# blackle/Megalania

Measured on AMD Instinct MI355X. Metric: SA neighbour-cost evals/s, higher is better.
Workload: dtype u64

## Files before the change

### megalania_amd/csrc/mgl_api.hip

```cpp
#include "mgl_kernels.hip"
#include "mgl_kernels2.hip"
#include "mgl_kernels3.hip"
#include "mgl_kernels4.hip"
#include "mgl_kernels5.hip"
#include "mgl_pbuild.hip"
#include "mgl_index.hip"
#include "mgl_matchfinder.hip"
#include "mgl_optimal.hip"
#include "mgl_adaptive.hip"
#include "mgl_props.hip"
#include "mgl_crossover.hip"
#include "../../include/megalania_hip.h"

#include <math.h>
#include <stdio.h>
#include <stdlib.h>
#include <string.h>
#include <string>
#include <vector>

static const uint16_t k_cost_table[2048] = {
#include "mgl_cost_table.inc"
};

// ... 86 lines not shown
	uint32_t chg_cap = MGL_CHG_CAP;
	uint32_t per_wave_pick, per_wave_rest, pick_waves;
	bool fuse;
	uint32_t fused_lds;
	size_t b2_bytes;
	BigScratch big;
	uint32_t* d_todo2;
	uint4* d_pickstate;
	uint4* d_pickrec;
	bool split_nbr, adaptive;
	bool form_single = false;
	uint32_t* d_counts;
	ApplyBuf ab;
	uint32_t apply_blocks;
	bool incremental_apply;
	bool snapshots;
	Base2 snap_lit, snap_best;
	SnapMeta* d_snap_meta;
	bool parallel_build;
	PBuild pb;
	hipEvent_t ev_begin, ev_end;
	std::vector<hipEvent_t> ev_pool;
	int accept_mode = MGL_ACCEPT_AUTO;
	uint32_t bulk_threshold = 0;
	bool bulk_now = true;
	uint64_t bulk_hold = 0;
	uint64_t blk_done = 0;
	uint64_t blk_imp0 = 0, blk_acc0 = 0;
	BulkBuf bulk;
	BatchBuf batch;
	bool batch_ok = false;
	uint32_t* d_strat_tgt = nullptr;
	uint32_t* d_strat_pre = nullptr;
	bool select_small = false;
	uint32_t* h_bstat = nullptr;
	hipEvent_t ev_bstat = nullptr;
	uint32_t force_xo_nomem = 0;
	uint32_t force_batch_fail = 0;
	uint32_t force_batch_late = 0;
	AcceptLimits lim, lim_max;
	uint64_t batch_early_giveups = 0;
	uint64_t batch_accepts = 0, batch_fallbacks = 0;
	std::vector<uint8_t> mode_log;
	uint32_t force_rollbacks = 0;
	uint64_t bulk_rollbacks = 0;
	bool best_unverified = false;
	uint32_t sim_waves = MGL_SIM_WAVES;
	std::vector<hipEvent_t> ev_sim_pool;
	int64_t time_sim_step = -1;
	bool count_traffic = false;
	unsigned long long* d_traffic = nullptr;
	uint32_t short_looks = 0;
	hipEvent_t ev_val = nullptr;
	int mf_finder = MGL_MF_NEAREST;
	uint32_t mf_depth = MGL_MF_DEF_DEPTH;
	uint32_t mf_built = 0;
	uint32_t* d_mf_off = nullptr;
	uint32_t* d_mf_src = nullptr;
	uint16_t* d_mf_len = nullptr;
	size_t mf_total = 0;
	double mf_ms = 0;
};

static uint64_t ceil_sqrt_u64(uint64_t x)
{
	uint64_t r = (uint64_t)sqrt((double)x);
// ... 194 lines not shown
	if (!sa->snapshots)
		hipLaunchKernelGGL(k_copy_best, dim3(256), dim3(256), 0, sa->stream, (const Control*)sa->base.ctl,
		                   (const mgl_pk*)sa->base.v.slab, sa->d_best, sa->ctx.n);
	hipLaunchKernelGGL(k_apply_chains, dim3(sa->apply_blocks), dim3(MGL_APPLY_THREADS), 0, sa->stream, sa->ctx, accept_b2(sa), sa->base.ctl, accept_ab(sa), sa->lim);
	hipLaunchKernelGGL(k_apply_jobs, dim3(1024), dim3(256), 0, sa->stream, sa->b2, (const Control*)sa->base.ctl, sa->ab, 0, (const uint32_t*)nullptr);
	hipLaunchKernelGGL(k_apply_jobs, dim3(1024), dim3(256), 0, sa->stream, sa->b2, (const Control*)sa->base.ctl, sa->ab, 1, (const uint32_t*)nullptr);
	hipLaunchKernelGGL(k_build_end, dim3(1), dim3(64), sa->build_lds, sa->stream, sa->ctx, sa->b2, sa->base.ctl, sa->snapshots ? 1 : 0, sa->d_counts, sa->adaptive ? 1 : 0, sa->form_single ? 1 : 0);
	HIPCHK(hipGetLastError());
	return MGL_OK;
}
static const bool g_trace = getenv("MGL_TRACE") != nullptr, g_prof_big = getenv("MGL_PROF_BIG") != nullptr;
#define NBR_TRACE(name) do { if (g_trace) { fprintf(stderr, "[mgl] %s\n", name); hipError_t e_ = hipDeviceSynchronize(); if (e_ != hipSuccess) fprintf(stderr, "[mgl] %s -> %s\n", name, hipGetErrorString(e_)); } } while (0)
static hipEvent_t sim_event(mgl_sa* sa, size_t i)
{
	while (sa->ev_sim_pool.size() <= i) {
		hipEvent_t e = nullptr;
		if (hipEventCreate(&e) != hipSuccess) return nullptr;
		sa->ev_sim_pool.push_back(e);
	}
	return sa->ev_sim_pool[i];
}
static uint32_t nbr_slices(const mgl_sa* sa)
{
	const uint32_t K = sa->cfg.neighbours_per_step;
	return (sa->halves >= 2 && K >= 1024) ? sa->halves : 1u;
}
static void launch_targets(mgl_sa* sa, hipStream_t st, uint64_t step_override)
{
	const uint32_t K = sa->cfg.neighbours_per_step;
	const uint64_t* onwalk = sa->incremental ? sa->b2.onwalk : sa->base.v.onwalk;
	const uint32_t nw0 = sa->incremental ? sa->b2.nw0 : (sa->ctx.n + 63u) >> 6;
	hipLaunchKernelGGL(k_rank_blocks, dim3(sa->ctx.strat_nblk), dim3(64), 0, st, onwalk, nw0, sa->d_strat_pre, sa->ctx.strat_nblk);
	hipLaunchKernelGGL(k_rank_scan, dim3(1), dim3(1024), 0, st, sa->d_strat_pre, sa->ctx.strat_nblk);
	hipLaunchKernelGGL(k_targets, dim3((K + 3u) / 4u), dim3(256), 0, st, sa->ctx, onwalk, nw0, (const Control*)sa->base.ctl, sa->cfg.seed, step_override, K, sa->d_strat_tgt);
}
static int launch_targets_ahead(mgl_sa* sa, uint64_t next_gstep)
{
	if (!sa->d_strat_pre || !sa->incremental) return MGL_OK;
	HIPCHK(hipEventRecord(sa->ev_tgt_go, sa->stream));
	HIPCHK(hipStreamWaitEvent(sa->stream2, sa->ev_tgt_go, 0));
	launch_targets(sa, sa->stream2, next_gstep);
	HIPCHK(hipEventRecord(sa->ev_tgt, sa->stream2));
	HIPCHK(hipGetLastError());
	sa->tgt_ahead = 1;
	return MGL_OK;
}
static int launch_neighbours(mgl_sa* sa, uint64_t step_override, bool zero_counts = true)
{
	const uint32_t K = sa->cfg.neighbours_per_step;
	if (sa->d_strat_pre) {
		if (sa->tgt_ahead) HIPCHK(hipStreamWaitEvent(sa->stream, sa->ev_tgt, 0));
		if (sa->tgt_ahead != 1) launch_targets(sa, sa->stream, step_override);
		sa->tgt_ahead = 0;
	}
	if (!sa->incremental) {
		const uint32_t blocks = (K + sa->waves_per_block - 1) / sa->waves_per_block;
		hipLaunchKernelGGL(k_neighbours, dim3(blocks), dim3(64 * sa->waves_per_block), sa->nbr_lds, sa->stream, sa->ctx, sa->base.v,
		                   (const Control*)sa->base.ctl, sa->cfg.seed, step_override, K, sa->nbr, sa->per_wave_bytes,
		                   (const uint32_t*)nullptr, (const uint32_t*)nullptr); NBR_TRACE("k_neighbours");
		HIPCHK(hipGetLastError());
		return MGL_OK;
	}
	if (zero_counts) HIPCHK(hipMemsetAsync(sa->d_counts, 0, 8 * sizeof(uint32_t), sa->stream));
	const uint32_t blocks2 = (K + sa->waves_per_block2 - 1) / sa->waves_per_block2;
	const bool split_now = sa->split_nbr && !sa->form_single;
	const uint32_t sim_lds_regular = ((((sa->ctx.L.total + 31u) >> 5) + 3u) & ~3u) * 4u + sa->chg_cap * 16u;
	if (split_now) {
		const uint32_t slices = nbr_slices(sa);
		HIPCHK(hipEventRecord(sa->ev_fork, sa->stream));
		if (slices >= 2) HIPCHK(hipStreamWaitEvent(sa->stream2, sa->ev_fork, 0));
#if !MGL_TAIL_EARLY
		HIPCHK(hipStreamWaitEvent(sa->stream3, sa->ev_fork, 0));
#endif
		for (uint32_t h = 0; h < slices; h++) {
			const uint32_t j0 = (uint32_t)((uint64_t)K * h / slices), j1 = (uint32_t)((uint64_t)K * (h + 1) / slices);
			hipStream_t st = (h & 1u) ? sa->stream2 : sa->stream;
			if (sa->fuse && !sa->d_prof) {
				hipLaunchKernelGGL((k_neighbours2<false, MGL_NBR_PICKWALK>), dim3(j1 - j0), dim3(64), sa->fused_lds, st, sa->ctx,
				                   sa->b2, sa->base.ctl, sa->cfg.seed, step_override, K, sa->nbr, sa->fused_lds, sa->d_todo, sa->d_counts,
				                   (unsigned long long*)nullptr, sa->big, sa->d_pickrec, j0, j1, sa->d_pickstate); NBR_TRACE("k_neighbours2<false, MGL_NBR_PICKWALK>");
				HIPCHK(hipEventRecord(sa->ev_rest[h], st));
				continue;
			}
			hipLaunchKernelGGL((sa->d_prof ? k_neighbours2<false, MGL_NBR_PICK, true> : k_neighbours2<false, MGL_NBR_PICK>), dim3((j1 - j0 + sa->pick_waves - 1) / sa->pick_waves), dim3(64 * sa->pick_waves),
			                   (MGL_PICK_T_GLOBAL ? 0u : 4096u) + sa->pick_waves * sa->per_wave_pick, st, sa->ctx,
			                   sa->b2, sa->base.ctl, sa->cfg.seed, step_override, K, sa->nbr, sa->per_wave_pick, sa->d_todo, sa->d_counts,
			                   sa->d_prof, sa->big, sa->d_pickrec, j0, j1, sa->d_pickstate); NBR_TRACE("k_neighbours2<false, MGL_NBR_PICK>");
			hipLaunchKernelGGL((k_neighbours2<false, MGL_NBR_REST>), dim3(j1 - j0), dim3(64), sa->per_wave_rest, st, sa->ctx,
			                   sa->b2, sa->base.ctl, sa->cfg.seed, step_override, K, sa->nbr, sa->per_wave_rest, sa->d_todo, sa->d_counts,
			                   g_prof_big ? (unsigned long long*)nullptr : sa->d_prof, sa->big, sa->d_pickrec, j0, j1, sa->d_pickstate); NBR_TRACE("k_neighbours2<false, MGL_NBR_REST>");
			HIPCHK(hipEventRecord(sa->ev_rest[h], st));
		}
		HIPCHK(hipGetLastError());
		for (uint32_t h = 0; h < slices; h++) {
			const uint32_t j0 = (uint32_t)((uint64_t)K * h / slices), j1 = (uint32_t)((uint64_t)K * (h + 1) / slices);
			HIPCHK(hipStreamWaitEvent(sa->stream3, sa->ev_rest[h], 0));
			if (sa->time_sim_step >= 0 && h < 2) HIPCHK(hipEventRecord(sim_event(sa, 4 * (size_t)sa->time_sim_step + 2 * h), sa->stream3));
			if (sa->count_traffic)
				hipLaunchKernelGGL(k_sim<true>, dim3(j1 - j0), dim3(64 * sa->sim_waves), sim_lds_regular, sa->stream3, sa->ctx, sa->b2, sa->base.ctl,
				                   sa->nbr, sa->big, j0, j1, sa->d_traffic);
			else
				hipLaunchKernelGGL(k_sim<false>, dim3(j1 - j0), dim3(64 * sa->sim_waves), sim_lds_regular, sa->stream3, sa->ctx, sa->b2, sa->base.ctl,
				                   sa->nbr, sa->big, j0, j1, (unsigned long long*)nullptr);
			NBR_TRACE("k_sim");
			if (sa->time_sim_step >= 0 && h < 2) HIPCHK(hipEventRecord(sim_event(sa, 4 * (size_t)sa->time_sim_step + 2 * h + 1), sa->stream3));
		}
		HIPCHK(hipEventRecord(sa->ev_sim, sa->stream3));
		for (uint32_t h = 1; h < slices; h += 2) HIPCHK(hipStreamWaitEvent(sa->stream, sa->ev_rest[h], 0));
	}
	if (!sa->split_nbr || sa->form_single) {
		hipLaunchKernelGGL((k_neighbours2<false, MGL_NBR_FULL>), dim3(blocks2), dim3(64 * sa->waves_per_block2), sa->nbr2_lds, sa->stream, sa->ctx,
		                   sa->b2, sa->base.ctl, sa->cfg.seed, step_override, K, sa->nbr, sa->per_wave2, sa->d_todo, sa->d_counts,
		                   sa->d_prof, sa->big, sa->d_pickrec, 0u, K, sa->d_pickstate); NBR_TRACE("k_neighbours2<false, MGL_NBR_FULL>");
	}
	const uint32_t bigblocks = sa->big.slots < 1024u ? sa->big.slots : 1024u;
	const uint32_t big_lds = 4096u + sa->per_wave2 + 12u * MGL_BIG_CAP + MGL_COOP_BYTES;
	hipLaunchKernelGGL((k_neighbours2<true, MGL_NBR_FULL>), dim3(bigblocks), dim3(64 * sa->big_waves), big_lds, sa->stream, sa->ctx,
	                   sa->b2, sa->base.ctl, sa->cfg.seed, step_override, K, sa->nbr, sa->per_wave2, sa->d_todo2, sa->d_counts + 1,
	                   g_prof_big ? sa->d_prof : (unsigned long long*)nullptr, sa->big, split_now ? sa->d_pickrec : (uint4*)nullptr, 0u, K, sa->d_pickstate); NBR_TRACE("k_neighbours2<true, MGL_NBR_FULL>");
#if !MGL_TAIL_EARLY
	if (split_now) HIPCHK(hipStreamWaitEvent(sa->stream, sa->ev_sim, 0));
#endif
	const uint32_t blocks = (K + sa->waves_per_block - 1) / sa->waves_per_block;
	hipLaunchKernelGGL(k_neighbours, dim3(blocks < 256u ? blocks : 256u), dim3(64 * sa->waves_per_block), sa->nbr_lds, sa->stream, sa->ctx, sa->base.v,
	                   (const Control*)sa->base.ctl, sa->cfg.seed, step_override, K, sa->nbr, sa->per_wave_bytes,
	                   (const uint32_t*)sa->d_todo2, (const uint32_t*)(sa->d_counts + 1)); NBR_TRACE("k_neighbours");
#if MGL_TAIL_EARLY
	if (split_now) HIPCHK(hipStreamWaitEvent(sa->stream, sa->ev_sim, 0));
// ... 12 lines not shown
static int export_slab(mgl_sa* sa, const mgl_pk* d_slab, mgl_packet* packets)
{
	hipLaunchKernelGGL(k_export, dim3(1024), dim3(256), 0, sa->stream, d_slab, sa->d_aos, sa->n);
	HIPCHK(hipGetLastError());
	HIPCHK(hipMemcpyAsync(packets, sa->d_aos, sizeof(mgl_packet) * (size_t)sa->n, hipMemcpyDeviceToHost, sa->stream));
	HIPCHK(hipStreamSynchronize(sa->stream));
	return MGL_OK;
}

extern "C" void mgl_sa_destroy(mgl_sa* sa)
{
	if (!sa) return;
	(void)hipSetDevice(sa->device);
	if (sa->stream) (void)hipStreamSynchronize(sa->stream);
	dfree(sa->d_data); dfree(sa->d_bucket_off); dfree(sa->d_bucket_pos); dfree(sa->d_bucket_nx); dfree(sa->d_quad_pos); dfree(sa->d_quad_nx); dfree(sa->d_cost_tbl);
	dfree(sa->d_quad_rank); dfree(sa->d_quad_run); dfree(sa->d_oct_pos);
	for (int i = 0; i < 6; i++) { if (i != 0 && i != 2) { dfree(sa->d_xpos[i]); dfree(sa->d_xrank[i]); dfree(sa->d_xrun[i]); } dfree(sa->d_xnxb[i]); } dfree(sa->d_oct_rank); dfree(sa->d_oct_run);
	dfree(sa->d_hex_pos); dfree(sa->d_hex_rank); dfree(sa->d_hex_run); dfree(sa->d_oct_nx8); dfree(sa->d_hex_nx8);
	free_base(sa->base); free_base(sa->scratch);
	if (!sa->snapshots) dfree(sa->d_best);
	dfree(sa->nbr.cost); dfree(sa->nbr.ndiffs); dfree(sa->nbr.walked); dfree(sa->nbr.win); dfree(sa->nbr.win2); dfree(sa->nbr.dpos);
	dfree(sa->bulk.ckey); dfree(sa->bulk.cwin); dfree(sa->bulk.taken); dfree(sa->bulk.cstate); dfree(sa->bulk.cflags); dfree(sa->bulk.hdr);
	dfree(sa->nbr.dold); dfree(sa->nbr.dnew);
	dfree(sa->d_aos); dfree(sa->d_cum); dfree(sa->d_final_probs);
	free_b2(sa->b2, false);
	free_b2(sa->snap_lit, true); free_b2(sa->snap_best, true); dfree(sa->d_snap_meta);
	dfree(sa->pb.exits); dfree(sa->pb.entry); dfree(sa->pb.gexits); dfree(sa->pb.gentry); dfree(sa->pb.gsum); dfree(sa->pb.ch_map); dfree(sa->pb.ch_vs); dfree(sa->pb.ch_pk); dfree(sa->pb.ch_state); dfree(sa->pb.tf_ctx); dfree(sa->pb.tf_dist); dfree(sa->pb.tf_pk);
	dfree(sa->pb.st_in); dfree(sa->pb.hist); dfree(sa->pb.stage); dfree(sa->pb.stage_n); dfree(sa->pb.stage_over); dfree(sa->pb.acc); dfree(sa->pb.seg_off); dfree(sa->pb.unres);
	dfree(sa->d_todo); dfree(sa->d_prof);
	dfree(sa->big.sim_hdr); dfree(sa->big.sim_keys); dfree(sa->big.sim_pos);
	dfree(sa->big.ins_key); dfree(sa->big.rem_key); dfree(sa->big.ins_pos); dfree(sa->big.rem_pos); dfree(sa->big.uctx);
	if (sa->h_bstat) (void)hipHostFree(sa->h_bstat);
	if (sa->ev_bstat) (void)hipEventDestroy(sa->ev_bstat);
	dfree(sa->big.cont); dfree(sa->d_traffic); dfree(sa->d_strat_pre); dfree(sa->d_strat_tgt);
	{
		BatchBuf& bt = sa->batch;
		dfree(bt.hdr); dfree(bt.cl); dfree(bt.jpos); dfree(bt.jnew); dfree(bt.jold); dfree(bt.st_ikey); dfree(bt.st_rkey); dfree(bt.st_ipos);
		dfree(bt.st_rpos); dfree(bt.ops); dfree(bt.ins_cl); dfree(bt.rem_cl); dfree(bt.acc); dfree(bt.runs);
		dfree(bt.cnt_i); dfree(bt.cnt_r); dfree(bt.off_i); dfree(bt.off_r); dfree(bt.cur_i); dfree(bt.cur_r); dfree(bt.touched);
		dfree(bt.bk_ipos); dfree(bt.bk_rpos); dfree(bt.bk_ibit); dfree(bt.bk_icl); dfree(bt.bk_rcl);
	}
	for (hipEvent_t e : sa->ev_sim_pool) if (e) (void)hipEventDestroy(e);
	dfree(sa->d_todo2); dfree(sa->d_counts); dfree(sa->d_pickrec); dfree(sa->d_pickstate);
	dfree(sa->lim.why); dfree(sa->ab.hdr); dfree(sa->ab.ins_key); dfree(sa->ab.rem_key); dfree(sa->ab.ins_pos); dfree(sa->ab.rem_pos);
	dfree(sa->ab.tctx); dfree(sa->ab.scratch_pos); dfree(sa->ab.scratch_ev);
	dfree(sa->ab.span_pos); dfree(sa->ab.span_ev); dfree(sa->ab.jobs_b); dfree(sa->ab.jobs_c);
	dfree(sa->d_mf_off); dfree(sa->d_mf_src); dfree(sa->d_mf_len);
	dfree(sa->d_topk_pk); dfree(sa->d_topk_cost); dfree(sa->d_small); dfree(sa->d_sub_offs); dfree(sa->d_sub_lens);
	for (hipEvent_t e : sa->ev_pool) (void)hipEventDestroy(e);
	if (sa->ev_begin) (void)hipEventDestroy(sa->ev_begin);
	if (sa->ev_end) (void)hipEventDestroy(sa->ev_end);
	if (sa->stream2) (void)hipStreamDestroy(sa->stream2);
	if (sa->stream3) (void)hipStreamDestroy(sa->stream3);
	for (auto& e : sa->ev_rest) if (e) (void)hipEventDestroy(e);
	if (sa->ev_sim) (void)hipEventDestroy(sa->ev_sim);
	if (sa->ev_val) (void)hipEventDestroy(sa->ev_val);
	if (sa->ev_fork) (void)hipEventDestroy(sa->ev_fork);
	if (sa->ev_tgt) (void)hipEventDestroy(sa->ev_tgt);
	if (sa->ev_tgt_go) (void)hipEventDestroy(sa->ev_tgt_go);
	if (sa->ev_join) (void)hipEventDestroy(sa->ev_join);
	if (sa->stream) (void)hipStreamDestroy(sa->stream);
	delete sa;
}

static int create_impl(mgl_sa* sa, const uint8_t* data, size_t n)
{
	HIPCHK(hipSetDevice(sa->device));
// ... 354 lines not shown
			}
		}
		if (getenv("MGL_SIMW")) { const int w = atoi(getenv("MGL_SIMW")); if (w == 1 || w == 2 || w == 4 || w == 8) sa->sim_waves = (uint32_t)w; }
		sa->adaptive = sa->split_nbr && getenv("MGL_NO_ADAPT") == nullptr;
		sa->form_single = !sa->split_nbr;
		sa->pick_waves = getenv("MGL_PICK_WAVES") ? (uint32_t)atoi(getenv("MGL_PICK_WAVES")) : 0u;
		if (sa->pick_waves != 1 && sa->pick_waves != 2 && sa->pick_waves != 4 && sa->pick_waves != 8) sa->pick_waves = 0;
		{
			uint32_t best_w = 1, best_resident = 0;
			for (uint32_t w = 1; w <= 8; w *= 2) {
				const uint32_t bytes = (MGL_PICK_T_GLOBAL ? 0u : 4096u) + w * sa->per_wave_pick;
				if (bytes > 160u * 1024u) break;
				const uint32_t resident = (160u * 1024u / ((bytes + 1279u) / 1280u * 1280u)) * w;
				if (resident > best_resident) { best_resident = resident; best_w = w; }
			}
			if (n > (1u << 20)) best_w = 1;
			if (sa->pick_waves == 0 || (MGL_PICK_T_GLOBAL ? 0u : 4096u) + sa->pick_waves * sa->per_wave_pick > 160u * 1024u) sa->pick_waves = best_w;
		}
		HIPCHK(hipFuncSetAttribute((const void*)k_sim<false>, hipFuncAttributeMaxDynamicSharedMemorySize, 96 * 1024));
		HIPCHK(hipFuncSetAttribute((const void*)k_sim<true>, hipFuncAttributeMaxDynamicSharedMemorySize, 96 * 1024));
		HIPCHK(hipMalloc(&sa->d_traffic, sizeof(unsigned long long) * 2));
		HIPCHK(hipMemset(sa->d_traffic, 0, sizeof(unsigned long long) * 2));
		HIPCHK(hipFuncSetAttribute((const void*)k_build, hipFuncAttributeMaxDynamicSharedMemorySize, (int)sa->build_lds));
		HIPCHK(hipFuncSetAttribute((const void*)k_build_end, hipFuncAttributeMaxDynamicSharedMemorySize, (int)sa->build_lds));
	}

	if (!(sa->cfg.flags & MGL_F_POSITION_TARGETS)) {
		sa->ctx.strat_nblk = (uint32_t)((n + 4095u) / 4096u);
		HIPCHK(hipMalloc(&sa->d_strat_pre, sizeof(uint32_t) * (sa->ctx.strat_nblk + 2u)));
		HIPCHK(hipMemset(sa->d_strat_pre, 0, sizeof(uint32_t) * (sa->ctx.strat_nblk + 2u)));
		sa->ctx.strat_pre = sa->d_strat_pre;
		HIPCHK(hipMalloc(&sa->d_strat_tgt, sizeof(uint32_t) * sa->cfg.neighbours_per_step));
		sa->ctx.strat_tgt = sa->d_strat_tgt;
	}
	sa->sqrt_thresh = ceil_sqrt_u64(sa->cfg.iters_per_epoch);
	sa->bulk_threshold = getenv("MGL_BULK_THRESHOLD") ? (uint32_t)atoi(getenv("MGL_BULK_THRESHOLD"))
	                     : sa->batch_ok ? 2u : (n <= (1u << 20) ? 16u : n <= (1u << 24) ? 32u : 128u);
	if (sa->bulk_threshold == 0) sa->bulk_threshold = 1;

	hipLaunchKernelGGL(k_fill_literal, dim3(1024), dim3(256), 0, sa->stream, sa->base.v.slab, sa->ctx.n);
	if (!sa->d_best) HIPCHK(hipMalloc(&sa->d_best, sizeof(mgl_pk) * n));
	hipLaunchKernelGGL(k_fill_literal, dim3(1024), dim3(256), 0, sa->stream, sa->d_best, sa->ctx.n);
	HIPCHK(hipGetLastError());
	int rc = rebuild_base(sa, 0);
	if (rc) return rc;
	if (sa->incremental && sa->snapshots && (rc = launch_snapshot(sa, sa->snap_lit, 0, 0, 0))) return rc;
	HIPCHK(hipStreamSynchronize(sa->stream));
	{
		Control c0;
		HIPCHK(hipMemcpy(&c0, sa->base.ctl, sizeof c0, hipMemcpyDeviceToHost));
		if (c0.error_flags) return fail(MGL_EDEVICE, "mgl_sa_create: building the base structures of the all-literal slab failed");
	}
	return MGL_OK;
}

extern "C" mgl_sa* mgl_sa_create(const uint8_t* data, size_t n, mgl_properties props, const mgl_sa_config* cfg)
{
	if (!data || n == 0 || !cfg) { fail(MGL_EINVAL, "mgl_sa_create: bad data/size/config"); return nullptr; }
	if (n > MGL_MAX_INPUT) { fail(MGL_EINVAL, "mgl_sa_create: input larger than 176 000 000 bytes is not supported"); return nullptr; }
	if (props.lc + props.lp > 4 || props.pb > 4 || props.lc > 8) { fail(MGL_EINVAL, "mgl_sa_create: unsupported lc/lp/pb"); return nullptr; }
	mgl_sa* sa = new (std::nothrow) mgl_sa();
	if (!sa) { fail(MGL_ENOMEM, "mgl_sa_create: out of host memory"); return nullptr; }
	sa->cfg = *cfg;
	sa->props = props;
	sa->n = (uint32_t)n;
	sa->device = cfg->device;
// ... 1337 lines not shown
	case 10: {
		uint32_t v[16];
		*bytes = sizeof v;
		if (cap_bytes < sizeof v) return fail(MGL_ERANGE, "mgl_debug_dump: buffer too small");
		HIPCHK(hipMemcpy(v, sa->d_counts + 8, sizeof(uint32_t) * 8, hipMemcpyDeviceToHost));
		HIPCHK(hipMemcpy(v + 8, sa->d_counts, sizeof(uint32_t) * 8, hipMemcpyDeviceToHost));
		memcpy(out, v, sizeof v);
		return MGL_OK;
	}
	case 14: src = sa->ab.hdr; sz = sa->ab.hdr ? sizeof(uint32_t) * 16 : 0; break;
	case 16: src = sa->base.ctl; sz = sizeof(Control); break;
	case 15: src = sa->d_pickrec; sz = sa->d_pickrec ? sizeof(uint4) * sa->cfg.neighbours_per_step : 0; break;
	case 18: src = sa->d_quad_pos; sz = sizeof(uint32_t) * (sa->n - 1); break;
	case 19: src = sa->d_quad_nx; sz = sizeof(uint16_t) * (sa->n - 1); break;
	case 12: src = sa->d_bucket_off; sz = sizeof(uint32_t) * 65537; break;
	case 13: src = sa->d_bucket_pos; sz = sizeof(uint32_t) * (sa->n - 1); break;
	case 30: case 31: case 32: case 33: case 34: case 35: src = sa->d_xpos[what - 30]; sz = sizeof(uint32_t) * (sa->n - 1); break;
	case 40: case 41: case 42: case 43: case 44: case 45: src = sa->d_xrank[what - 40]; sz = src ? sizeof(uint32_t) * (sa->n - 1) : 0; break;
	case 50: case 51: case 52: case 53: case 54: case 55: src = sa->d_xrun[what - 50]; sz = src ? sizeof(uint32_t) * (sa->n - 1) : 0; break;
	case 60: case 61: case 62: case 63: case 64: case 65: src = sa->d_xnxb[what - 60]; sz = sa->n - 1; break;
	case 70: src = sa->d_oct_pos; sz = sizeof(uint32_t) * (sa->n - 1); break;
	case 71: src = sa->d_oct_rank; sz = sizeof(uint32_t) * (sa->n - 1); break;
	case 72: src = sa->d_oct_run; sz = sizeof(uint32_t) * (sa->n - 1); break;
	case 73: src = sa->d_oct_nx8; sz = sizeof(uint64_t) * (sa->n - 1); break;
	case 74: src = sa->d_hex_pos; sz = sizeof(uint32_t) * (sa->n - 1); break;
	case 75: src = sa->d_hex_rank; sz = sizeof(uint32_t) * (sa->n - 1); break;
	case 76: src = sa->d_hex_run; sz = sizeof(uint32_t) * (sa->n - 1); break;
	case 77: src = sa->d_hex_nx8; sz = sizeof(uint64_t) * (sa->n - 1); break;
	case 23: src = sa->nbr.cost; sz = sizeof(uint64_t) * sa->cfg.neighbours_per_step; break;
	case 24: src = sa->nbr.ndiffs; sz = sizeof(uint32_t) * sa->cfg.neighbours_per_step; break;
	case 25: src = sa->nbr.walked; sz = sizeof(uint32_t) * sa->cfg.neighbours_per_step; break;
	case 22: src = sa->nbr.win2; sz = sizeof(uint32_t) * sa->cfg.neighbours_per_step; break;
	case 21: src = sa->nbr.win; sz = sizeof(uint32_t) * 2 * sa->cfg.neighbours_per_step; break;
	case 11: src = sa->pb.acc; sz = sa->pb.acc ? sizeof(unsigned long long) * 8 : 0; break;
	default: return fail(MGL_EINVAL, "mgl_debug_dump: unknown selector");
	}
	*bytes = sz;
	if (sz > cap_bytes) return fail(MGL_ERANGE, "mgl_debug_dump: buffer too small");
	HIPCHK(hipMemcpy(out, src, sz, hipMemcpyDeviceToHost));
	if (what == 84) HIPCHK(hipMemset(sa->lim.why, 0, sizeof(uint32_t)));
	return MGL_OK;
}

extern "C" int mgl_debug_set(mgl_sa* sa, uint32_t key, uint64_t value)
{
	if (sa && key == 5) {
		sa->force_batch_late = (uint32_t)(value >> 32);
		sa->force_batch_fail = (uint32_t)value;
		if (sa->force_batch_late && !sa->force_batch_fail) sa->force_batch_fail = 1;
		return MGL_OK;
	}
	if (sa && key == 6) {
		const uint32_t id = (uint32_t)(value & 0xFFu);
		const uint64_t v = value >> 8;
		if (!sa->incremental || !sa->lim.why) return fail(MGL_EINVAL, "mgl_debug_set: no in-place accept on this handle");
		HIPCHK(hipSetDevice(sa->device));
		HIPCHK(hipStreamSynchronize(sa->stream));
		if (id == 0) {
			if (v) return fail(MGL_EINVAL, "mgl_debug_set: limit id 0 takes value 0 (restore the defaults)");
			for (uint32_t i = 1; i < MGL_LIM_COUNT; i++) sa->lim.v[i] = i == MGL_LIM_SOFT_REACH ? 0u : sa->lim_max.v[i];
		} else {
			if (id >= MGL_LIM_COUNT || v > sa->lim_max.v[id]) return fail(MGL_EINVAL, "mgl_debug_set: unknown limit, or a value above the compiled / allocated one");
			sa->lim.v[id] = (uint32_t)v;
		}
		HIPCHK(hipMemset(sa->lim.why, 0, sizeof(uint32_t)));
		return MGL_OK;
	}
	if (sa && key == 4) {
		if (!sa->d_traffic) return fail(MGL_EINVAL, "mgl_debug_set: no split neighbour evaluation on this handle");
		sa->count_traffic = value != 0;
		return MGL_OK;
	}
	if (!sa) return fail(MGL_EINVAL, "null handle");
	if (key == 0) { sa->ctx.diag_stop = (uint32_t)value; return MGL_OK; }
	if (key == 1) { sa->pb.force_fix = (uint32_t)value; return MGL_OK; }
	if (key == 2) {
		if (value < 8 || value > sa->chg_cap || (value & 7u)) return fail(MGL_EINVAL, "mgl_debug_set: list capacity must be a multiple of 8 within the allocated one");
		sa->big.chg_cap = (uint32_t)value;
		return MGL_OK;
	}
	if (key == 7) {
		if (value != 1 && value != 2 && value != MGL_BIG_WAVES) return fail(MGL_EINVAL, "mgl_debug_set: 1, 2 or MGL_BIG_WAVES wavefronts");
		sa->big_waves = (uint32_t)value;
		return MGL_OK;
	}
	if (key == 8) { sa->force_xo_nomem = (uint32_t)value; return MGL_OK; }
	if (key == 3) { sa->force_rollbacks = (uint32_t)value; return MGL_OK; }
	return fail(MGL_EINVAL, "mgl_debug_set: unknown key");
}

#include "mgl_exchange.inc"
```

### megalania_amd/csrc/mgl_kernels2.hip

```cpp
#include "mgl_base2.h"


struct BitAcc {
	uint32_t word;
	uint64_t bits;
};
__device__ __forceinline__ void bitacc_move(BitAcc& a, uint64_t* arr, uint32_t new_word, uint32_t lane)
{
	if (new_word == a.word) return;
	if (lane == 0) arr[a.word] = a.bits;
	for (uint32_t z = a.word + 1 + lane; z < new_word; z += 64) arr[z] = 0;
	a.word = new_word; a.bits = 0;
}

__device__ void build_body(const DevCtx& c, const Base2& b, Control* ctl, int check_cost)
{
	extern __shared__ __attribute__((aligned(16))) unsigned char smem[];
	uint16_t* T = (uint16_t*)smem;
	uint16_t* probs = (uint16_t*)(smem + 4096);
	uint32_t* cnt = (uint32_t*)(smem + 4096 + (size_t)b.ck_elems * 2);
	uint32_t* off = cnt + b.ck_elems;
	const uint32_t lane = threadIdx.x;
	const uint32_t total = c.L.total;
	if (check_cost && !ctl->accepted_flag) return;
// ... 826 lines not shown
	if (c.diag_stop == 1) { if (lane == 0) { out.cost[j] = MGL_INVALID_COST; out.ndiffs[j] = 0; out.walked[j] = first; } return; }
	if (MODE == MGL_NBR_REST && FUSED) {
		mutated = (hand->flags & MGL_HAND_MUTATED) != 0; second_set = (hand->flags & MGL_HAND_SECOND) != 0;
		if (mutated) {
			m_first = hand->m_first; m_second = hand->m_second;
			journal_set(jn, pos, first, m_first, lane);
			if (second_set) journal_set(jn, pos + 1, hand->second, m_second, lane);
		}
	} else if (!(BIG && resumed) && pos + 1 < c.n && (nbr_draw(rng) % 2u) == 0) {
		const mgl_pk second = uni64(b.slab[pos + 1]);
		const uint32_t ft = mgl_pk_type(first), flen = mgl_pk_len(first);
		const uint32_t st = mgl_pk_type(second), slen = mgl_pk_len(second), sdist = mgl_pk_dist(second);
		if ((ft == MGL_LONG_REP || ft == MGL_MATCH) && flen > 2) {
			m_second = mgl_pack(ft, mgl_pk_dist(first), flen - 1);
			m_first = MGL_PK_LITERAL;
			if (MODE == MGL_NBR_PICK && FUSED) hand->second = uni64(second);
			if (MODE != MGL_NBR_PICK) { journal_set(jn, pos, first, m_first, lane); journal_set(jn, pos + 1, second, m_second, lane); }
			second_set = true; mutated = true;
		} else if ((ft == MGL_LITERAL || ft == MGL_SHORT_REP) && (st == MGL_MATCH || st == MGL_LONG_REP)) {
			uint32_t rep_start = pos - (st == MGL_LONG_REP ? mgl_dist_at(&nb, sdist) : sdist);
			if (slen < MGL_MAX_MATCH && rep_start > 0 && rep_start <= pos && win_byte(win, pos) == c.data[rep_start - 1]) {
				m_first = mgl_pack(st, sdist, slen + 1);
				if (MODE != MGL_NBR_PICK) journal_set(jn, pos, first, m_first, lane);
				mutated = true;
			}
		}
	}
	enum { P_MODEL, P_SIM, P_TOPK, P_WALK, P_OUT };
	uint32_t phase = mutated ? P_WALK : P_MODEL;
	if (MODE == MGL_NBR_PICK && FUSED) {
		hand->m_first = uni64(m_first); hand->m_second = uni64(m_second); hand->rng_n = uni(rng.n);
		hand->flags = (mutated ? MGL_HAND_MUTATED : 0u) | (second_set ? MGL_HAND_SECOND : 0u);
	}
	if (MODE == MGL_NBR_PICK && mutated) return;
	TopkPlan plan;
	if (MODE == MGL_NBR_PICK) {
		if (PROF) pick_prof_mark(&pp, 0, lane);
		if (MGL_PICK_BATCH) topk_plan_make(plan, c, nb, lane);
		if (PROF) pick_prof_mark(&pp, 1, lane);
	}
	if (MODE == MGL_NBR_REST && c.diag_stop != 0 && c.diag_stop != 4 && c.diag_stop < 40) return;
	bool pick_is_mutation = !mutated;
	uint32_t pick_pos = pos;
	mgl_pk pick_inc = first;
	bool pick_best = false;
	bool have_pick = false;
	mgl_pk picked_pk = 0, resume_old = 0;
	uint32_t sim_limit = MGL_POS_INF;
	bool sim_overlay = false;
	int64_t delta = 0;
	bool generate_failed = false, sim_deferred = false, walk_long = false;
	uint32_t npicks = 0;
	uint32_t count = 0;
	uint32_t walked = 0;
	uint32_t wend = 0;
	uint32_t wsoft = 0xFFFFFFFFu, taint = 0xFu, dep = 0u;
	bool first_packet = true;
	uint32_t guard = 0;
	if (BIG && resumed) {
		bs.pos = uni(crec[9]); bs.ctx_state = uni(crec[10]);
		bs.dists[0] = uni(crec[11]); bs.dists[1] = uni(crec[12]); bs.dists[2] = uni(crec[13]); bs.dists[3] = uni(crec[14]);
		count = uni(crec[15]); walked = uni(crec[16]); npicks = uni(crec[17]); wsoft = uni(crec[18]); taint = uni(crec[19]); dep = uni(crec[20]);
		rng.n = uni(crec[21]); guard = uni(crec[22]); jn.count = uni(crec[23]); ch.n_ins = uni(crec[24]); ch.n_rem = uni(crec[25]);
		const uint32_t fl = uni(crec[26]);
		pick_best = (fl & 1u) != 0; second_set = (fl & 2u) != 0;
		pick_inc = (mgl_pk)uni(crec[28]) | ((mgl_pk)uni(crec[29]) << 32);
		resume_old = (mgl_pk)uni(crec[30]) | ((mgl_pk)uni(crec[31]) << 32);
// ... 304 lines not shown
		if (lane == 0) {
			out.dpos[(size_t)j * MGL_MAX_DIFFS + nd] = jn.pos[i];
			out.dold[(size_t)j * MGL_MAX_DIFFS + nd] = jn.old[i];
			out.dnew[(size_t)j * MGL_MAX_DIFFS + nd] = jn.neu[i];
		}
		nd++;
	}
	if (lane == 0) { if (!sim_deferred) out.cost[j] = total; out.ndiffs[j] = nd; out.walked[j] = walked; out.win[2u * j] = pos; out.win[2u * j + 1u] = wend; out.win2[j] = (wsoft < wend ? wsoft : wend) | (dep << 31); }
	if (prof_acc && lane == 0)
		prof_acc[32 + j] = ((__builtin_readcyclecounter() - t_begin) & 0xFFFFFFFFFFull) |
		                   ((unsigned long long)((ch.n_ins + ch.n_rem) & 0xFFFu) << 40) | ((unsigned long long)(walked & 0xFFFu) << 52);
}

template <bool BIG, int MODE, bool PROF = false>
__global__ void __launch_bounds__((MODE == MGL_NBR_PICK ? 512 : (BIG ? 64 * MGL_BIG_WAVES : 64)), (MODE == MGL_NBR_FULL ? (BIG ? 1 : MGL_NBR_WAVES_PER_SIMD) : (MODE == MGL_NBR_REST ? MGL_REST_WAVES_PER_SIMD : 4)))  k_neighbours2(DevCtx c, Base2 b, Control* ctl, uint64_t seed,
                                                     uint64_t step_override, uint32_t K, NbrOut out, uint32_t per_wave_bytes,
                                                     uint32_t* todo, uint32_t* todo_count, unsigned long long* prof_acc,
                                                     BigScratch big, uint4* pickrec, uint32_t j_base, uint32_t j_end, uint4* pickstate)
{
	const uint32_t waves = blockDim.x >> 6;
	if (BIG && blockIdx.x >= *big.todo_in_count) return;
	extern __shared__ __attribute__((aligned(16))) unsigned char smem[];
	uint16_t* T = (uint16_t*)smem;
	if (BIG && threadIdx.x == 0) { CoopCmd* cmd = coop_cmd(smem, per_wave_bytes); cmd->gen = 0; cmd->op = MGL_COOP_SIM; }
	if ((MODE == MGL_NBR_PICK || MODE == MGL_NBR_PICKWALK) && MGL_PICK_T_GLOBAL) {
		T = const_cast<uint16_t*>(c.cost_tbl);
	} else if (MODE != MGL_NBR_REST) {
		for (uint32_t i = threadIdx.x; i < 256; i += blockDim.x) reinterpret_cast<uint4*>(T)[i] = reinterpret_cast<const uint4*>(c.cost_tbl)[i];
		__syncthreads();
	}
	const uint32_t lane = threadIdx.x & 63u, wid = threadIdx.x >> 6;
	if constexpr (MODE == MGL_NBR_PICKWALK) {
		static_assert(!BIG && !PROF, "the fused instance is a regular launch without stage marks");
		PickHand hand;
		hand.target = 0; hand.rng_n = 0; hand.ctx_state = 0; hand.dists[0] = hand.dists[1] = hand.dists[2] = hand.dists[3] = 0;
		hand.first = hand.second = hand.m_first = hand.m_second = 0; hand.flags = 0;
		nbr2_one<false, MGL_NBR_PICK, false, true>(c, b, ctl, seed, step_override, K, out, per_wave_bytes, todo, todo_count, nullptr, big, pickrec, j_base, j_end, pickstate, smem, T,
		                                           blockIdx.x, lane, 0u, &hand);
		wave_sync();
		nbr2_one<false, MGL_NBR_REST, false, true>(c, b, ctl, seed, step_override, K, out, per_wave_bytes, todo, todo_count, nullptr, big, pickrec, j_base, j_end, pickstate, smem, T,
		                                           blockIdx.x, lane, 0u, &hand);
	} else if (BIG) {
		if (wid != 0) { coop_helpers(c, b, big, prof_acc, smem, per_wave_bytes, T, lane, wid); return; }
		const uint32_t n = *big.todo_in_count;
		for (uint32_t unit = blockIdx.x; unit < n; unit += gridDim.x)
			nbr2_one<BIG, MODE, PROF>(c, b, ctl, seed, step_override, K, out, per_wave_bytes, todo, todo_count, prof_acc, big, pickrec, j_base, j_end, pickstate, smem, T, unit, lane, 0u);
		if (lane == 0) { CoopCmd* cmd = coop_cmd(smem, per_wave_bytes); cmd->op = MGL_COOP_EXIT; cmd->gen = cmd->gen + 1u; }
		__syncthreads();
	} else {
		nbr2_one<BIG, MODE, PROF>(c, b, ctl, seed, step_override, K, out, per_wave_bytes, todo, todo_count, prof_acc, big, pickrec, j_base, j_end, pickstate, smem, T,
		                    blockIdx.x * waves + wid, lane, wid);
	}
}


#ifndef MGL_SIM_WAVES
#define MGL_SIM_WAVES 2u
#endif
#define MGL_SIM_WAVES_MAX 8u
struct SimShared {
	uint16_t* T;
	uint32_t* dyn;
	unsigned long long* sum;
	uint32_t* nu_many;
};
template <bool COUNT>
__device__ __forceinline__ void sim_one(const DevCtx& c, const Base2& b, Control* ctl, const NbrOut& out, const BigScratch& big, const uint4* hdrs,
                                        uint32_t j, const SimShared& sh, unsigned long long* traffic_ctr)
{
	const uint4 hdr = hdrs[j];
	if (hdr.x == 0xFFFFFFFFu) return;
	const uint32_t cap = big.chg_cap;
	uint32_t* s_bits = sh.dyn;
	uint32_t* s_pos = sh.dyn + ((((c.L.total + 31u) >> 5) + 3u) & ~3u);
// ... 61 lines not shown


__global__ void __launch_bounds__(64) k_rank_blocks(const uint64_t* onwalk, uint32_t nw0, uint32_t* pre, uint32_t nblk)
{
	const uint32_t blk = blockIdx.x, lane = threadIdx.x;
	if (blk >= nblk) return;
	const uint32_t w = blk * 64u + lane;
	unsigned long long v = w < nw0 ? (unsigned long long)__popcll(onwalk[w]) : 0ull;
	v = wave_sum64(v);
	if (lane == 0) pre[blk + 1u] = (uint32_t)v;
}
__global__ void __launch_bounds__(1024) k_rank_scan(uint32_t* pre, uint32_t nblk)
{
	__shared__ uint32_t s_w[16], s_base;
	const uint32_t tid = threadIdx.x, lane = tid & 63u, wid = tid >> 6;
	if (tid == 0) { s_base = 0; pre[0] = 0; }
	__syncthreads();
	for (uint32_t base = 0; base < nblk; base += blockDim.x) {
		const uint32_t i = base + tid;
		const uint32_t v = i < nblk ? pre[i + 1u] : 0u;
		uint32_t incl = v;
		for (int o = 1; o < 64; o <<= 1) { const uint32_t t = (uint32_t)__shfl_up((int)incl, o, 64); if ((int)lane >= o) incl += t; }
		if (lane == 63) s_w[wid] = incl;
		__syncthreads();
		uint32_t bsum = s_base;
		for (uint32_t q = 0; q < wid; q++) bsum += s_w[q];
		if (i < nblk) pre[i + 1u] = bsum + incl;
		__syncthreads();
		if (tid == blockDim.x - 1u) s_base = bsum + incl;
		__syncthreads();
	}
}

__global__ void __launch_bounds__(256) k_targets(DevCtx c, const uint64_t* onwalk, uint32_t nw0, const Control* ctl, uint64_t seed, uint64_t step_override,
                                                 uint32_t K, uint32_t* tgt)
{
	const uint32_t j = blockIdx.x * (blockDim.x >> 6) + (threadIdx.x >> 6), lane = threadIdx.x & 63u;
	if (j >= K) return;
	const uint64_t gstep = step_override != ~0ull ? step_override : ctl->gstep;
	const uint32_t t = stratified_target(onwalk, nw0, c.strat_pre, c.strat_nblk, c.strat_pre[c.strat_nblk], K, j, mgl_rng_draw(mgl_rng_key(seed, gstep, j), 0), lane);
	if (lane == 0) tgt[j] = t;
}
```

Baseline: 15.87 million.

## Predict picking neighbours and launch them first in fused neighbour kernel

Adds a cheap prediction in k_targets of whether each neighbour will take the expensive pick path, then a k_pick_order kernel that partitions each slice so predicted-picking neighbours come first in block order. The fused PICKWALK kernel reads this permutation to map block index to neighbour unit, aiming to schedule long-running blocks early and reduce tail imbalance. It costs an extra slab read per target, an extra kernel launch, and per-step scans, and it changes the pickstate argument semantics in the fused path.

```diff
diff --git a/megalania_amd/csrc/mgl_api.hip b/megalania_amd/csrc/mgl_api.hip
--- a/megalania_amd/csrc/mgl_api.hip
+++ b/megalania_amd/csrc/mgl_api.hip
@@ -142,6 +142,8 @@
 	bool batch_ok = false;
 	uint32_t* d_strat_tgt = nullptr;
 	uint32_t* d_strat_pre = nullptr;
+	unsigned char* d_pick_hint = nullptr;
+	uint32_t* d_pick_order = nullptr;
 	bool select_small = false;
 	uint32_t* h_bstat = nullptr;
 	hipEvent_t ev_bstat = nullptr;
@@ -402,7 +404,12 @@
 	const uint32_t nw0 = sa->incremental ? sa->b2.nw0 : (sa->ctx.n + 63u) >> 6;
 	hipLaunchKernelGGL(k_rank_blocks, dim3(sa->ctx.strat_nblk), dim3(64), 0, st, onwalk, nw0, sa->d_strat_pre, sa->ctx.strat_nblk);
 	hipLaunchKernelGGL(k_rank_scan, dim3(1), dim3(1024), 0, st, sa->d_strat_pre, sa->ctx.strat_nblk);
-	hipLaunchKernelGGL(k_targets, dim3((K + 3u) / 4u), dim3(256), 0, st, sa->ctx, onwalk, nw0, (const Control*)sa->base.ctl, sa->cfg.seed, step_override, K, sa->d_strat_tgt);
+	hipLaunchKernelGGL(k_targets, dim3((K + 3u) / 4u), dim3(256), 0, st, sa->ctx, sa->b2, onwalk, nw0, (const Control*)sa->base.ctl, sa->cfg.seed, step_override, K, sa->d_strat_tgt,
+	                   sa->d_pick_hint);
+	if (sa->d_pick_order) {
+		const uint32_t slices = nbr_slices(sa);
+		hipLaunchKernelGGL(k_pick_order, dim3(slices), dim3(1024), 0, st, (const unsigned char*)sa->d_pick_hint, sa->d_pick_order, K, slices);
+	}
 }
 static int launch_targets_ahead(mgl_sa* sa, uint64_t next_gstep)
 {
@@ -443,12 +450,12 @@
 		HIPCHK(hipStreamWaitEvent(sa->stream3, sa->ev_fork, 0));
 #endif
 		for (uint32_t h = 0; h < slices; h++) {
-			const uint32_t j0 = (uint32_t)((uint64_t)K * h / slices), j1 = (uint32_t)((uint64_t)K * (h + 1) / slices);
+			const uint32_t j0 = mgl_slice_bound(K, h, slices), j1 = mgl_slice_bound(K, h + 1, slices);
 			hipStream_t st = (h & 1u) ? sa->stream2 : sa->stream;
 			if (sa->fuse && !sa->d_prof) {
 				hipLaunchKernelGGL((k_neighbours2<false, MGL_NBR_PICKWALK>), dim3(j1 - j0), dim3(64), sa->fused_lds, st, sa->ctx,
 				                   sa->b2, sa->base.ctl, sa->cfg.seed, step_override, K, sa->nbr, sa->fused_lds, sa->d_todo, sa->d_counts,
-				                   (unsigned long long*)nullptr, sa->big, sa->d_pickrec, j0, j1, sa->d_pickstate); NBR_TRACE("k_neighbours2<false, MGL_NBR_PICKWALK>");
+				                   (unsigned long long*)nullptr, sa->big, sa->d_pickrec, j0, j1, (uint4*)sa->d_pick_order); NBR_TRACE("k_neighbours2<false, MGL_NBR_PICKWALK>");
 				HIPCHK(hipEventRecord(sa->ev_rest[h], st));
 				continue;
 			}
@@ -463,7 +470,7 @@
 		}
 		HIPCHK(hipGetLastError());
 		for (uint32_t h = 0; h < slices; h++) {
-			const uint32_t j0 = (uint32_t)((uint64_t)K * h / slices), j1 = (uint32_t)((uint64_t)K * (h + 1) / slices);
+			const uint32_t j0 = mgl_slice_bound(K, h, slices), j1 = mgl_slice_bound(K, h + 1, slices);
 			HIPCHK(hipStreamWaitEvent(sa->stream3, sa->ev_rest[h], 0));
 			if (sa->time_sim_step >= 0 && h < 2) HIPCHK(hipEventRecord(sim_event(sa, 4 * (size_t)sa->time_sim_step + 2 * h), sa->stream3));
 			if (sa->count_traffic)
@@ -542,7 +549,7 @@
 	dfree(sa->big.ins_key); dfree(sa->big.rem_key); dfree(sa->big.ins_pos); dfree(sa->big.rem_pos); dfree(sa->big.uctx);
 	if (sa->h_bstat) (void)hipHostFree(sa->h_bstat);
 	if (sa->ev_bstat) (void)hipEventDestroy(sa->ev_bstat);
-	dfree(sa->big.cont); dfree(sa->d_traffic); dfree(sa->d_strat_pre); dfree(sa->d_strat_tgt);
+	dfree(sa->big.cont); dfree(sa->d_traffic); dfree(sa->d_strat_pre); dfree(sa->d_strat_tgt); dfree(sa->d_pick_hint); dfree(sa->d_pick_order);
 	{
 		BatchBuf& bt = sa->batch;
 		dfree(bt.hdr); dfree(bt.cl); dfree(bt.jpos); dfree(bt.jnew); dfree(bt.jold); dfree(bt.st_ikey); dfree(bt.st_rkey); dfree(bt.st_ipos);
@@ -963,6 +970,11 @@
 		sa->ctx.strat_pre = sa->d_strat_pre;
 		HIPCHK(hipMalloc(&sa->d_strat_tgt, sizeof(uint32_t) * sa->cfg.neighbours_per_step));
 		sa->ctx.strat_tgt = sa->d_strat_tgt;
+		if (sa->incremental && sa->split_nbr && getenv("MGL_NO_ORDER") == nullptr) {
+			HIPCHK(hipMalloc(&sa->d_pick_hint, sa->cfg.neighbours_per_step));
+			HIPCHK(hipMemset(sa->d_pick_hint, 1, sa->cfg.neighbours_per_step));
+			HIPCHK(hipMalloc(&sa->d_pick_order, sizeof(uint32_t) * sa->cfg.neighbours_per_step));
+		}
 	}
 	sa->sqrt_thresh = ceil_sqrt_u64(sa->cfg.iters_per_epoch);
 	sa->bulk_threshold = getenv("MGL_BULK_THRESHOLD") ? (uint32_t)atoi(getenv("MGL_BULK_THRESHOLD"))
@@ -2366,12 +2378,15 @@
 	case 25: src = sa->nbr.walked; sz = sizeof(uint32_t) * sa->cfg.neighbours_per_step; break;
 	case 22: src = sa->nbr.win2; sz = sizeof(uint32_t) * sa->cfg.neighbours_per_step; break;
 	case 21: src = sa->nbr.win; sz = sizeof(uint32_t) * 2 * sa->cfg.neighbours_per_step; break;
+	case 26: src = sa->d_pick_hint; sz = src ? sa->cfg.neighbours_per_step : 0; break;
+	case 27: src = sa->d_pick_order; sz = src ? sizeof(uint32_t) * sa->cfg.neighbours_per_step : 0; break;
+	case 28: src = sa->d_pickstate; sz = src ? sizeof(uint4) * 2 * sa->cfg.neighbours_per_step : 0; break;
 	case 11: src = sa->pb.acc; sz = sa->pb.acc ? sizeof(unsigned long long) * 8 : 0; break;
 	default: return fail(MGL_EINVAL, "mgl_debug_dump: unknown selector");
 	}
 	*bytes = sz;
 	if (sz > cap_bytes) return fail(MGL_ERANGE, "mgl_debug_dump: buffer too small");
-	HIPCHK(hipMemcpy(out, src, sz, hipMemcpyDeviceToHost));
+	if (sz) HIPCHK(hipMemcpy(out, src, sz, hipMemcpyDeviceToHost));
 	if (what == 84) HIPCHK(hipMemset(sa->lim.why, 0, sizeof(uint32_t)));
 	return MGL_OK;
 }
@@ -2419,6 +2434,24 @@
 		return MGL_OK;
 	}
 	if (key == 8) { sa->force_xo_nomem = (uint32_t)value; return MGL_OK; }
+	if (key == 9) {
+		if (!sa->d_pick_order) return fail(MGL_EINVAL, "mgl_debug_set: no launch order on this handle");
+		const uint32_t K = sa->cfg.neighbours_per_step, slices = nbr_slices(sa);
+		std::vector<unsigned char> h(K);
+		uint64_t x = value;
+		for (uint32_t j = 0; j < K; j++) {
+			x = x * 6364136223846793005ull + 1442695040888963407ull;
+			h[j] = value == 0 ? 0 : value == 1 ? 1 : value == 2 ? (unsigned char)(j & 1u) : (unsigned char)((x >> 40) % 3u);
+		}
+		HIPCHK(hipSetDevice(sa->device));
+		HIPCHK(hipStreamSynchronize(sa->stream));
+		HIPCHK(hipStreamSynchronize(sa->stream2));
+		HIPCHK(hipMemcpy(sa->d_pick_hint, h.data(), K, hipMemcpyHostToDevice));
+		hipLaunchKernelGGL(k_pick_order, dim3(slices), dim3(1024), 0, sa->stream, (const unsigned char*)sa->d_pick_hint, sa->d_pick_order, K, slices);
+		HIPCHK(hipGetLastError());
+		HIPCHK(hipStreamSynchronize(sa->stream));
+		return MGL_OK;
+	}
 	if (key == 3) { sa->force_rollbacks = (uint32_t)value; return MGL_OK; }
 	return fail(MGL_EINVAL, "mgl_debug_set: unknown key");
 }
diff --git a/megalania_amd/csrc/mgl_kernels2.hip b/megalania_amd/csrc/mgl_kernels2.hip
--- a/megalania_amd/csrc/mgl_kernels2.hip
+++ b/megalania_amd/csrc/mgl_kernels2.hip
@@ -882,7 +882,10 @@
 		hand->m_first = uni64(m_first); hand->m_second = uni64(m_second); hand->rng_n = uni(rng.n);
 		hand->flags = (mutated ? MGL_HAND_MUTATED : 0u) | (second_set ? MGL_HAND_SECOND : 0u);
 	}
-	if (MODE == MGL_NBR_PICK && mutated) return;
+	if (MODE == MGL_NBR_PICK && mutated) {
+		if (!FUSED && lane == 0) reinterpret_cast<uint32_t*>(pickstate)[8u * j + 7u] = 1u;
+		return;
+	}
 	TopkPlan plan;
 	if (MODE == MGL_NBR_PICK) {
 		if (PROF) pick_prof_mark(&pp, 0, lane);
@@ -1253,14 +1256,16 @@
 	const uint32_t lane = threadIdx.x & 63u, wid = threadIdx.x >> 6;
 	if constexpr (MODE == MGL_NBR_PICKWALK) {
 		static_assert(!BIG && !PROF, "the fused instance is a regular launch without stage marks");
+		const uint32_t* const order = reinterpret_cast<const uint32_t*>(pickstate);
+		const uint32_t unit = order != nullptr ? order[j_base + blockIdx.x] - j_base : blockIdx.x;
 		PickHand hand;
 		hand.target = 0; hand.rng_n = 0; hand.ctx_state = 0; hand.dists[0] = hand.dists[1] = hand.dists[2] = hand.dists[3] = 0;
 		hand.first = hand.second = hand.m_first = hand.m_second = 0; hand.flags = 0;
-		nbr2_one<false, MGL_NBR_PICK, false, true>(c, b, ctl, seed, step_override, K, out, per_wave_bytes, todo, todo_count, nullptr, big, pickrec, j_base, j_end, pickstate, smem, T,
-		                                           blockIdx.x, lane, 0u, &hand);
+		nbr2_one<false, MGL_NBR_PICK, false, true>(c, b, ctl, seed, step_override, K, out, per_wave_bytes, todo, todo_count, nullptr, big, pickrec, j_base, j_end, nullptr, smem, T,
+		                                           unit, lane, 0u, &hand);
 		wave_sync();
-		nbr2_one<false, MGL_NBR_REST, false, true>(c, b, ctl, seed, step_override, K, out, per_wave_bytes, todo, todo_count, nullptr, big, pickrec, j_base, j_end, pickstate, smem, T,
-		                                           blockIdx.x, lane, 0u, &hand);
+		nbr2_one<false, MGL_NBR_REST, false, true>(c, b, ctl, seed, step_override, K, out, per_wave_bytes, todo, todo_count, nullptr, big, pickrec, j_base, j_end, nullptr, smem, T,
+		                                           unit, lane, 0u, &hand);
 	} else if (BIG) {
 		if (wid != 0) { coop_helpers(c, b, big, prof_acc, smem, per_wave_bytes, T, lane, wid); return; }
 		const uint32_t n = *big.todo_in_count;
@@ -1388,12 +1393,71 @@
 	}
 }
 
-__global__ void __launch_bounds__(256) k_targets(DevCtx c, const uint64_t* onwalk, uint32_t nw0, const Control* ctl, uint64_t seed, uint64_t step_override,
-                                                 uint32_t K, uint32_t* tgt)
+__device__ __forceinline__ bool nbr_will_pick(const DevCtx& c, const Base2& b, uint32_t pos, uint64_t key)
+{
+	if (pos >= c.n || pos + 1 >= c.n || (mgl_rng_draw(key, 1) % 2u) != 0) return true;
+	const mgl_pk first = b.slab[pos], second = b.slab[pos + 1];
+	const uint32_t ft = mgl_pk_type(first), flen = mgl_pk_len(first);
+	const uint32_t st = mgl_pk_type(second), slen = mgl_pk_len(second), sdist = mgl_pk_dist(second);
+	if ((ft == MGL_LONG_REP || ft == MGL_MATCH) && flen > 2) return false;
+	if ((ft == MGL_LITERAL || ft == MGL_SHORT_REP) && (st == MGL_MATCH || st == MGL_LONG_REP)) {
+		uint32_t d = sdist;
+		if (st == MGL_LONG_REP) { const mgl_wstate nb = base_state_at(b, pos); d = mgl_dist_at(&nb, sdist); }
+		const uint32_t rep_start = pos - d;
+		if (slen < MGL_MAX_MATCH && rep_start > 0 && rep_start <= pos && c.data[pos] == c.data[rep_start - 1]) return false;
+	}
+	return true;
+}
+
+__global__ void __launch_bounds__(256) k_targets(DevCtx c, Base2 b, const uint64_t* onwalk, uint32_t nw0, const Control* ctl, uint64_t seed, uint64_t step_override,
+                                                 uint32_t K, uint32_t* tgt, unsigned char* hint)
 {
 	const uint32_t j = blockIdx.x * (blockDim.x >> 6) + (threadIdx.x >> 6), lane = threadIdx.x & 63u;
 	if (j >= K) return;
 	const uint64_t gstep = step_override != ~0ull ? step_override : ctl->gstep;
-	const uint32_t t = stratified_target(onwalk, nw0, c.strat_pre, c.strat_nblk, c.strat_pre[c.strat_nblk], K, j, mgl_rng_draw(mgl_rng_key(seed, gstep, j), 0), lane);
+	const uint64_t key = mgl_rng_key(seed, gstep, j);
+	const uint32_t t = stratified_target(onwalk, nw0, c.strat_pre, c.strat_nblk, c.strat_pre[c.strat_nblk], K, j, mgl_rng_draw(key, 0), lane);
 	if (lane == 0) tgt[j] = t;
-}
+	if (hint != nullptr) {
+		const bool picks = nbr_will_pick(c, b, t, key);
+		if (lane == 0) hint[j] = picks ? 1 : 0;
+	}
+}
+
+__host__ __device__ __forceinline__ uint32_t mgl_slice_bound(uint32_t K, uint32_t h, uint32_t slices) { return (uint32_t)((uint64_t)K * h / slices); }
+
+__device__ __forceinline__ uint32_t block_rank(bool flag, uint32_t* s_w, uint32_t* total)
+{
+	const uint32_t lane = threadIdx.x & 63u, wid = threadIdx.x >> 6;
+	const unsigned long long m = __ballot(flag);
+	__syncthreads();
+	if (lane == 0) s_w[wid] = (uint32_t)__popcll(m);
+	__syncthreads();
+	uint32_t below = 0, all = 0;
+	for (uint32_t q = 0; q < 16u; q++) { const uint32_t v = s_w[q]; if (q < wid) below += v; all += v; }
+	*total = all;
+	return below + (uint32_t)__popcll(m & ((1ull << lane) - 1ull));
+}
+__global__ void __launch_bounds__(1024) k_pick_order(const unsigned char* hint, uint32_t* order, uint32_t K, uint32_t slices)
+{
+	__shared__ uint32_t s_w[16];
+	const uint32_t j0 = mgl_slice_bound(K, blockIdx.x, slices), j1 = mgl_slice_bound(K, blockIdx.x + 1u, slices);
+	uint32_t picking = 0;
+	for (uint32_t s = j0; s < j1; s += 1024u) {
+		const uint32_t j = s + threadIdx.x;
+		uint32_t t;
+		(void)block_rank(j < j1 && hint[j] != 0, s_w, &t);
+		picking += t;
+	}
+	uint32_t front_seen = 0, back_seen = 0;
+	for (uint32_t s = j0; s < j1; s += 1024u) {
+		const uint32_t j = s + threadIdx.x;
+		const bool in = j < j1, front = in && hint[j] != 0;
+		uint32_t tf;
+		const uint32_t rf = block_rank(front, s_w, &tf);
+		if (front) order[j0 + front_seen + rf] = j;
+		else if (in) order[j0 + picking + back_seen + (threadIdx.x - rf)] = j;
+		const uint32_t n_in = j1 - s < 1024u ? j1 - s : 1024u;
+		front_seen += tf; back_seen += n_in - tf;
+	}
+}
```

New measurement: 16.45 million, median of 6. +3.7%, better.
